# superyuri/FinRL

Hardware: AMD Instinct MI355X
Metric: env-steps/sec at N parallel envs (DOW30, 8 indicators) (higher is better)
Workload: dtype f64

## Files before the change

finrl_amd/csrc/finenv_stocknp.hip:

```cpp

#include <hip/hip_runtime.h>
#include <stdint.h>
#include <stdio.h>
#include <stdlib.h>
#include <string.h>

#include "finenv.h"
#include "finenv_dev.h"
#include "finenv_host.h"

namespace {

constexpr int kWave = 64;
constexpr int kMaxN = FINENV_STOCKNP_MAX_TICKERS;
constexpr int kRowA = kMaxN + 1;
constexpr int kRowH = 2 * kMaxN + 1;
constexpr int kWaves = 4;
constexpr int kLdsPerWave = kWave * kRowH + 2 * kMaxN * kWave + kMaxN;

struct NpParams {
    finenv_stocknp_config cfg;
    finenv_stocknp_panel panel;
    finenv_stocknp_state st;
    const float *actions;
    float *obs;
    float *reward;
    uint8_t *done;
    float *term_obs;
    const uint8_t *mask;
    int32_t auto_reset;
    int32_t D;
    int32_t obs_pitch;
    uint32_t magicN;
    unsigned long long *dbg;
    int32_t diag;
    int32_t *win;
};
struct NpParamsHist : NpParams {
    finenv_stocknp_history hist;
};
template <bool HIST>
using NpArgs = typename std::conditional<HIST, NpParamsHist, NpParams>::type;

#ifdef FINENV_DIAG
#define NDIAG(bit) (p.diag & (bit))
#else
#define NDIAG(bit) 0
#endif

#define NF(fld) (*at(p.st.f64, (unsigned)(fld) * (unsigned)E + (unsigned)e))
#define NI(fld) (*at(p.st.i32, (unsigned)(fld) * (unsigned)E + (unsigned)e))
#define NS(k, i) (*at(p.st.f32, ((unsigned)(k) * (unsigned)N + (unsigned)(i)) * (unsigned)E + (unsigned)e))
#define NWIN(r) (*at(p.win, (unsigned)(r) * (unsigned)E + (unsigned)e))

struct Num { double v; int tag; };
__device__ __forceinline__ Num mk(double v, int tag) { Num r; r.v = v; r.tag = tag; return r; }
__device__ __forceinline__ int promote(int a, int b)
{
    return a == FINENV_NT_PY ? b : (b == FINENV_NT_PY ? a : max(a, b));
}
__device__ __forceinline__ Num n_add(Num a, Num b)
{
    const int t = promote(a.tag, b.tag);
    const double r32 = (double)((float)a.v + (float)b.v), r64 = a.v + b.v;
    return mk(t == FINENV_NT_F32 ? r32 : r64, t);
}
__device__ __forceinline__ Num n_sub(Num a, Num b)
{
    const int t = promote(a.tag, b.tag);
    const double r32 = (double)((float)a.v - (float)b.v), r64 = a.v - b.v;
    return mk(t == FINENV_NT_F32 ? r32 : r64, t);
}
__device__ __forceinline__ Num n_mul(Num a, Num b)
{
    const int t = promote(a.tag, b.tag);
    const double r32 = (double)((float)a.v * (float)b.v), r64 = a.v * b.v;
    return mk(t == FINENV_NT_F32 ? r32 : r64, t);
}
__device__ __forceinline__ Num n_div(Num a, Num b)
{
    const int t = promote(a.tag, b.tag);
    const double r32 = (double)((float)a.v / (float)b.v), r64 = a.v / b.v;
    return mk(t == FINENV_NT_F32 ? r32 : r64, t);
}
__device__ __forceinline__ double floordiv_f32(float a, float b, double q)
{
    const double r = fma(-q, (double)b, (double)a);
    const float mod = (float)((a < 0.0f && r != 0.0) ? r - (double)b : r);
    float div = (a - mod) / b;
    if (mod < 0.0f) div -= 1.0f;
    float fl = floorf(div);
    if (div - fl > 0.5f) fl += 1.0f;
    return (double)fl;
}
__device__ __forceinline__ Num n_floordiv(Num a, Num b)
{
    const int t = promote(a.tag, b.tag);
    const double av = (t == FINENV_NT_F32) ? (double)(float)a.v : a.v;
    const double q = floordiv_true(av, b.v);
    if (t == FINENV_NT_F32 && fabs(q) >= 0x1p22) return mk(floordiv_f32((float)av, (float)b.v, q), t);
    return mk(q, t);
}

__device__ __forceinline__ int scaled_action(float action, float max_stock)
{
    constexpr float kS = 2147483520.0f;
    return (int)__builtin_amdgcn_fmed3f(action * max_stock, -kS, kS);
}

template <bool kCompact = false>
__device__ __forceinline__ void np_write_rows(float *__restrict__ dst, const NpParams &p, int e0,
                                              int nenv_w, int row_day,
                                              unsigned long long lane_mask, const float *heads,
                                              int lane, int k_lo = 0, int k_hi = 1 << 30)
{
    const int N = p.cfg.n_tickers, D = p.D;
    const int pitch = dst == p.obs ? p.obs_pitch : D;
    write_obs_rows_generic<8, 16, kCompact>(
        dst, p.panel.obs_tmpl, D, e0, nenv_w, row_day, lane_mask, heads, kRowH, lane,
        [=](int day, int col) { return day * D + col; },
        [=](int col) {
            const int hidx = col - 3 - N;
            return col == 0 ? 0 : ((hidx >= 0 && hidx < 2 * N) ? 1 + hidx : -1);
        }, k_lo, k_hi, pitch);
}

__device__ __forceinline__ float holdings_value(const float *scol, const float *__restrict__ price,
                                                unsigned pb, int N, const float *prow = nullptr)
{
    if (prow != nullptr) {
        auto prodl = [&](int i) { return scol[i * kWave] * prow[i]; };
        float suml;
        if (N < 8) {
            suml = 0.0f;
            for (int i = 0; i < N; ++i) suml += prodl(i);
        } else {
            float r8[8];
#pragma unroll
            for (int j = 0; j < 8; ++j) r8[j] = prodl(j);
            const int full = N - (N & 7);
            for (int i = 8; i < full; i += 8) {
#pragma unroll
                for (int j = 0; j < 8; ++j) r8[j] += prodl(i + j);
            }
            suml = ((r8[0] + r8[1]) + (r8[2] + r8[3])) + ((r8[4] + r8[5]) + (r8[6] + r8[7]));
            for (int i = full; i < N; ++i) suml += prodl(i);
        }
        return suml;
    }
    auto prod = [&](int i) { return scol[i * kWave] * *at(price, pb + (unsigned)i); };
    float sum;
    if (N < 8) {
        sum = 0.0f;
        for (int i = 0; i < N; ++i) sum += prod(i);
    } else {
        float r8[8];
#pragma unroll
        for (int j = 0; j < 8; ++j) r8[j] = prod(j);
        const int full = N - (N & 7);
        for (int i = 8; i < full; i += 8) {
#pragma unroll
            for (int j = 0; j < 8; ++j) r8[j] += prod(i + j);
        }
        sum = ((r8[0] + r8[1]) + (r8[2] + r8[3])) + ((r8[4] + r8[5]) + (r8[6] + r8[7]));
        for (int i = full; i < N; ++i) sum += prod(i);
    }
    return sum;
}

template <bool RESET_ONLY, bool WIN = false, bool HIST = false>
__global__ void __launch_bounds__(kWave *kWaves *(RESET_ONLY ? 1 : 2)) stocknp_kernel(const NpArgs<HIST> p)
{
    static_assert(!(HIST && RESET_ONLY), "the record is taken by the step");
    __shared__ float lds_all[kWaves * (kLdsPerWave + (HIST ? 2 * kWave : 0))];
    const int lane = threadIdx.x & (kWave - 1);
    const int wib = (threadIdx.x >> 6) % kWaves;
    const int role = (threadIdx.x >> 6) / kWaves;
    float *heads = lds_all + wib * kLdsPerWave;
    float *stk = heads + kWave * kRowH;
    float *cdl = stk + kMaxN * kWave;
    const int E = p.cfg.n_envs, N = p.cfg.n_tickers;
    const int e0 = (blockIdx.x * kWaves + wib) * kWave;
    if (e0 >= E) return;
    const int nenv_w = min(kWave, E - e0);
    const bool valid = lane < nenv_w;
    const int e = valid ? e0 + lane : e0;
    float *scol = stk + lane, *ccol = cdl + lane;
    float *head = heads + lane * kRowH;
    float *prow_lds = cdl + kMaxN * kWave;
    int *hpark = reinterpret_cast<int *>(lds_all + kWaves * kLdsPerWave) + wib * 2 * kWave;

    auto do_reset = [&](Num &amount, Num &ta, Num &gr, Num &ita, int row = 0) {
        for (int i = 0; i < N; ++i) {
            scol[i * kWave] = NS(2, i);
            ccol[i * kWave] = 0.0f;
        }
        amount = mk(NF(FINENV_NF_AMOUNT0), NI(FINENV_NI_AMOUNT0_TAG));
        const unsigned rpb = WIN ? (unsigned)(row * N) : 0u;
        ta = n_add(amount, mk((double)holdings_value(scol, p.panel.price, rpb, N), FINENV_NT_F32));
        ita = ta;
        gr = mk(0.0, FINENV_NT_PY);
    };
    auto fill_head = [&](Num amount) {
        const double fl = p.cfg.obs_amount_floor;
        const Num shown = (fl > 0.0 && fl > amount.v) ? mk(fl, FINENV_NT_PY) : amount;
        head[0] = (float)n_mul(shown, mk(0x1p-12, FINENV_NT_PY)).v;
        for (int i = 0; i < N; ++i) {
            head[1 + i] = scol[i * kWave] * 0x1p-6f;
            head[1 + N + i] = ccol[i * kWave];
        }
    };
    auto store_books = [&](int i_lo, int i_hi) {
        for (int i = i_lo; i < i_hi; ++i) {
            NS(0, i) = scol[i * kWave];
            NS(1, i) = ccol[i * kWave];
        }
    };
    auto store_state = [&](Num amount, Num ta, Num gr, Num ita, int rtag, int day, int i_lo = 0,
                           int i_hi = 1 << 30) {
        NF(FINENV_NF_AMOUNT) = amount.v;
        NF(FINENV_NF_TOTAL_ASSET) = ta.v;
        NF(FINENV_NF_GAMMA_REWARD) = gr.v;
        NF(FINENV_NF_INITIAL_TOTAL_ASSET) = ita.v;
        NI(FINENV_NI_TAGS) = amount.tag | (ta.tag << 2) | (gr.tag << 4) | (ita.tag << 6) | (rtag << 8);
        NI(FINENV_NI_DAY) = day;
        store_books(i_lo, min(i_hi, N));
    };

    if (RESET_ONLY) {
        const bool sel = valid && (p.mask == nullptr || p.mask[e] != 0);
        Num amount, ta, gr, ita;
        int row0 = 0;
        if (WIN) {
            const int ps = NWIN(0), pt = NWIN(1);
            row0 = min(max(ps, 0), p.cfg.n_days - 1);
            if (sel) {
                NWIN(2) = ps;
                NWIN(3) = pt;
            }
        }
        do_reset(amount, ta, gr, ita, row0);
        if (sel) store_state(amount, ta, gr, ita, (NI(FINENV_NI_TAGS) >> 8) & 3, row0);
        if (p.obs == nullptr) return;
        fill_head(amount);
        wave_sync();
        np_write_rows(p.obs, p, e0, nenv_w, row0, __ballot(sel), heads, lane);
        return;
    }

    const int kpatch = (2 + 3 * N) / kWave + 1;
    auto head_widx = [N](int col) {
        const int hidx = col - 3 - N;
        return col == 0 ? 0 : ((hidx >= 0 && hidx < 2 * N) ? 1 + hidx : -1);
    };
    typedef float np_f4 __attribute__((ext_vector_type(4)));
    typedef np_f4 np_f4u __attribute__((aligned(4)));
    const int lpr = 16 * kpatch;
    const bool quad_ok = kpatch <= 2 && p.D >= kWave * kpatch;
    auto head_quads = [&](const np_f4 hq, int el_lo, int el_hi) {
        const int rpi = kWave / lpr, sub = lane / lpr, q = lane & (lpr - 1);
        int w[4];
#pragma unroll
        for (int u = 0; u < 4; ++u) w[u] = head_widx(4 * q + u);
        char *const hb = reinterpret_cast<char *>(p.obs + (size_t)e0 * p.obs_pitch);
        constexpr int kB = 8;
        const int hi = min(nenv_w, el_hi);
        for (int g0 = el_lo / rpi; g0 * rpi < hi; g0 += kB) {
            float pv4[kB][4];
#pragma unroll
            for (int j = 0; j < kB; ++j) {
                const int el = min((g0 + j) * rpi + sub, kWave - 1);
#pragma unroll
                for (int u = 0; u < 4; ++u) pv4[j][u] = heads[el * kRowH + (w[u] >= 0 ? w[u] : 0)];
            }
#pragma unroll
            for (int j = 0; j < kB; ++j) {
                const int el = (g0 + j) * rpi + sub;
                if (el >= hi) continue;
                np_f4 v;
#pragma unroll
                for (int u = 0; u < 4; ++u) v[u] = w[u] >= 0 ? pv4[j][u] : hq[u];
                *reinterpret_cast<np_f4u *>(hb + (size_t)((unsigned)(el * p.obs_pitch + 4 * q) * 4u)) = v;
            }
        }
    };
    auto head_quad_load = [&](int row) -> np_f4 {
        return *reinterpret_cast<const np_f4u *>(reinterpret_cast<const char *>(p.panel.obs_tmpl) +
                                                 (size_t)((unsigned)(row * p.D + 4 * (lane & (lpr - 1))) * 4u));
    };
    if (role == 0) STAMP64(0);
    if (role == 1) {
        int day_s = NI(FINENV_NI_DAY) + 1;
        int last_s = p.cfg.n_days - 1;
        if constexpr (HIST) {
            int hlen_s = *at(p.hist.len, (unsigned)e), hfl_s = *at(p.hist.flags, (unsigned)e);
            if constexpr (WIN) {
                last_s = win_last_day(p.win + 2 * (size_t)E, E, e, p.cfg.n_days);
                asm volatile("s_waitcnt vmcnt(0)"
                             : "+v"(day_s), "+v"(last_s), "+v"(hlen_s), "+v"(hfl_s) : : "memory");
                day_s = min(max(day_s, 0), p.cfg.n_days - 1);
            } else {
                asm volatile("s_waitcnt vmcnt(0)" : "+v"(day_s), "+v"(hlen_s), "+v"(hfl_s) : : "memory");
            }
            hpark[lane] = hlen_s;
            hpark[kWave + lane] = hfl_s;
        } else if constexpr (WIN) {
            last_s = win_last_day(p.win + 2 * (size_t)E, E, e, p.cfg.n_days);
            asm volatile("s_waitcnt vmcnt(0)" : "+v"(day_s), "+v"(last_s) : : "memory");
            day_s = min(max(day_s, 0), p.cfg.n_days - 1);
        } else {
            asm volatile("s_waitcnt vmcnt(0)" : "+v"(day_s) : : "memory");
        }
        lds_barrier();
        const bool done_s = day_s == last_s;
        const unsigned long long vm = __ballot(valid), dm = __ballot(done_s && valid);
        if (dm != 0ull && p.term_obs != nullptr)
            np_write_rows<true>(p.term_obs, p, e0, nenv_w, day_s, dm, heads, lane, kpatch);
        int rd = (done_s && p.auto_reset) ? 0 : day_s;
        if (WIN && p.auto_reset && dm != 0ull) {
            const int ps = win_start(p.win, e, p.cfg.n_days);
            if (done_s) rd = ps;
        }
        const int rd0 = __builtin_amdgcn_readfirstlane(rd);
        const bool same_row = __all(!valid || rd == rd0);
        const bool share = quad_ok && dm == 0ull && same_row;
        np_f4 hq = {0.0f, 0.0f, 0.0f, 0.0f};
        if (share) hq = head_quad_load(rd0);
        STAMP64(9);
        const int c0 = kpatch * kWave, span = p.D - c0;
        if (same_row && span >= 4) {
            const int nq = (span + 3) >> 2;
            char *const ob = reinterpret_cast<char *>(p.obs + (size_t)e0 * p.obs_pitch);
            for (int q0 = 0; q0 < nq; q0 += kWave) {
                const bool qa = q0 + lane < nq;
                const int start = qa ? min(c0 + 4 * (q0 + lane), p.D - 4) : c0;
                const np_f4 t = *reinterpret_cast<const np_f4u *>(
                    reinterpret_cast<const char *>(p.panel.obs_tmpl) + (size_t)((unsigned)(rd0 * p.D + start) * 4u));
#pragma unroll 4
                for (int el = 0; el < nenv_w; ++el)
                    if (qa) *reinterpret_cast<np_f4u *>(ob + (size_t)((unsigned)(el * p.obs_pitch + start) * 4u)) = t;
            }
        } else {
            np_write_rows(p.obs, p, e0, nenv_w, rd, vm, heads, lane, kpatch);
        }
        STAMP64(10);
        lds_barrier();
        if (share && !NDIAG(1)) {
            head_quads(hq, kWave / 2, kWave);
            if (valid) store_books(N / 2, N);
        }
        return;
    }
    int day_ld = NI(FINENV_NI_DAY) + 1;
    int w_last = p.cfg.n_days - 1;
    if (WIN) {
        w_last = win_last_day(p.win + 2 * (size_t)E, E, e, p.cfg.n_days);
        day_ld = min(max(day_ld, 0), p.cfg.n_days - 1);
    }
    const int day = day_ld;
    const int tags = NI(FINENV_NI_TAGS);
    Num amount = mk(NF(FINENV_NF_AMOUNT), tags & 3);
    const Num ta_old = mk(NF(FINENV_NF_TOTAL_ASSET), (tags >> 2) & 3);
    Num gr = mk(NF(FINENV_NF_GAMMA_REWARD), (tags >> 4) & 3);
    Num ita = mk(NF(FINENV_NF_INITIAL_TOTAL_ASSET), (tags >> 6) & 3);
    float sv[kMaxN], cv[kMaxN], av[kMaxN];
#pragma unroll
    for (int i = 0; i < kMaxN; ++i) {
        sv[i] = NS(0, min(i, N - 1));
        cv[i] = NS(1, min(i, N - 1));
    }
    const int a_total = nenv_w * N;
    const float *const a_src = p.actions + (size_t)e0 * N;
#pragma unroll
    for (int j = 0; j < kMaxN; ++j) {
        const int f = j * kWave + lane;
        av[j] = *at(a_src, (unsigned)(f < a_total ? f : a_total - 1));
    }
    const unsigned pb = (unsigned)(day * N);
    const int day0 = __builtin_amdgcn_readfirstlane(day);
    const bool uni = __all(day == day0);
    float prv = 0.0f;
    if (uni && lane < kMaxN) prv = *at(p.panel.price, (unsigned)(day0 * N + min(lane, N - 1)));
    const float *prow = uni ? prow_lds : nullptr;
    np_f4 head_q = {0.0f, 0.0f, 0.0f, 0.0f};
    if (quad_ok) head_q = head_quad_load(day0);
    const bool calm = *at(p.panel.turb_bool, (unsigned)day) == 0.0f;
    lds_barrier();
#pragma unroll
    for (int j = 0; j < kMaxN; ++j) {
        const int f = j * kWave + lane;
        if (f < a_total) {
            const int el = (N == 1) ? f : (int)__umulhi((unsigned)f, p.magicN);
            heads[el * kRowA + (f - el * N)] = av[j];
        }
    }
#pragma unroll
    for (int i = 0; i < kMaxN; ++i) {
        if (i >= N) continue;
        cv[i] += 1.0f;
        scol[i * kWave] = sv[i];
        ccol[i * kWave] = cv[i];
    }
    if (uni && lane < kMaxN) prow_lds[lane] = prv;
    wave_sync();
    STAMP64(1);
    const float *arow = heads + lane * kRowA;
    const float ms = (float)p.cfg.max_stock;
    const Num one_m = mk(1 - p.cfg.sell_cost_pct, FINENV_NT_PY);
    const Num one_p = mk(1 + p.cfg.buy_cost_pct, FINENV_NT_PY);
    const int min_action = p.cfg.min_action;

    constexpr int kPB = 8;
    bool head_filled = false;
    if (__all(amount.tag == FINENV_NT_F64)) {
        double amt = amount.v;
        float (&sr)[kMaxN] = sv, (&cr)[kMaxN] = cv;
        float pr_[kMaxN];
        int ai[kMaxN];
#pragma unroll
        for (int i = 0; i < kMaxN; ++i) {
            const int ic = min(i, N - 1);
            ai[i] = scaled_action(arow[ic], ms);
            pr_[i] = 0.0f;
        }
        if (uni) {
#pragma unroll
            for (int i = 0; i < kMaxN; ++i) pr_[i] = prow_lds[min(i, N - 1)];
        } else {
#pragma unroll
            for (int i = 0; i < kMaxN; ++i) pr_[i] = *at(p.panel.price, pb + (unsigned)min(i, N - 1));
        }
        STAMP64(11);
#pragma unroll
        for (int i = 0; i < kMaxN; ++i) {
            if (i >= N) continue;
            const int a = ai[i];
            const float pr = pr_[i];
            const bool ok = calm && a < -min_action && pr > 0.0f;
            const float s = sr[i];
            const double want = (double)(-a);
            const bool is_int = want < (double)s;
            const double sell = is_int ? want : (double)s;
            const float s_new = (float)((double)s - sell);
            const double t64 = ((double)pr * sell) * one_m.v;
            const double t32 = (double)((pr * (float)sell) * (float)one_m.v);
            const double amt_new = amt + (is_int ? t64 : t32);
            sr[i] = ok ? s_new : s;
            cr[i] = ok ? 0.0f : cr[i];
            amt = ok ? amt_new : amt;
        }
        STAMP64(7);
        double xr[kMaxN];
#pragma unroll
        for (int i = 0; i < kMaxN; ++i) {
            const double d = (double)pr_[i];
            const double x = __builtin_amdgcn_rcp(d);
            xr[i] = fma(fma(-d, x, 1.0), x, x);
        }
        STAMP64(12);
#pragma unroll
        for (int i = 0; i < kMaxN; ++i) {
            if (i >= N) continue;
            const int a = ai[i];
            const double d = (double)pr_[i];
            const bool ok = calm && a > min_action && pr_[i] > 0.0f;
            double q = floor(amt * xr[i]);
            const double r = fma(-q, d, amt);
            q += (r < 0.0) ? -1.0 : ((r >= d) ? 1.0 : 0.0);
            const double buy = ((double)a < q) ? (double)a : q;
            const float s_new = (float)((double)sr[i] + buy);
            const double amt_new = amt - ((d * buy) * one_p.v);
            sr[i] = ok ? s_new : sr[i];
            cr[i] = ok ? 0.0f : cr[i];
            amt = ok ? amt_new : amt;
        }
        amount = mk(amt, FINENV_NT_F64);
        STAMP64(8);
        wave_sync();
        {
            const double fl = p.cfg.obs_amount_floor;
            const Num shown = (fl > 0.0 && fl > amount.v) ? mk(fl, FINENV_NT_PY) : amount;
            head[0] = (float)n_mul(shown, mk(0x1p-12, FINENV_NT_PY)).v;
        }
#pragma unroll
        for (int i = 0; i < kMaxN; ++i) {
            if (i >= N) continue;
            scol[i * kWave] = sr[i];
            ccol[i * kWave] = cr[i];
            head[1 + i] = sr[i] * 0x1p-6f;
            head[1 + N + i] = cr[i];
        }
        head_filled = calm;
    } else {
        for (int i0 = 0; i0 < N; i0 += kPB) {
            float prb[kPB];
    #pragma unroll
            for (int j = 0; j < kPB; ++j) prb[j] = 0.0f;
            if (uni) {
#pragma unroll
                for (int j = 0; j < kPB; ++j) prb[j] = prow_lds[min(i0 + j, N - 1)];
            } else {
#pragma unroll
                for (int j = 0; j < kPB; ++j)
                    prb[j] = *at(p.panel.price, pb + (unsigned)min(i0 + j, N - 1));
            }
    #pragma unroll
            for (int j = 0; j < kPB; ++j) pin(prb[j]);
    #pragma unroll
            for (int j = 0; j < kPB; ++j) {
            const int i = i0 + j;
            if (i >= N) break;
            const int a = scaled_action(arow[i], ms);
            const float pr = prb[j];
            if (calm && a < -min_action && pr > 0.0f) {
                const float s = scol[i * kWave];
                const double want = (double)(-a);
                const bool is_int = want < (double)s;
                const double sell = is_int ? want : (double)s;
                scol[i * kWave] = (float)((double)s - sell);
                const Num t0 = is_int ? mk((double)pr * sell, FINENV_NT_F64)
                                      : mk((double)(pr * (float)sell), FINENV_NT_F32);
                amount = n_add(amount, n_mul(t0, one_m));
                ccol[i * kWave] = 0.0f;
            }
            }
        }
        for (int i0 = 0; i0 < N; i0 += kPB) {
            float prb[kPB];
    #pragma unroll
            for (int j = 0; j < kPB; ++j) prb[j] = 0.0f;
            if (uni) {
#pragma unroll
                for (int j = 0; j < kPB; ++j) prb[j] = prow_lds[min(i0 + j, N - 1)];
            } else {
#pragma unroll
                for (int j = 0; j < kPB; ++j)
                    prb[j] = *at(p.panel.price, pb + (unsigned)min(i0 + j, N - 1));
            }
    #pragma unroll
            for (int j = 0; j < kPB; ++j) pin(prb[j]);
    #pragma unroll
            for (int j = 0; j < kPB; ++j) {
            const int i = i0 + j;
            if (i >= N) break;
            const int a = scaled_action(arow[i], ms);
            const float pr = prb[j];
            if (calm && a > min_action && pr > 0.0f) {
                const Num q = n_floordiv(amount, mk((double)pr, FINENV_NT_F32));
                const bool is_int = (double)a < q.v;
                const double buy = is_int ? (double)a : q.v;
                const Num t0 = is_int ? mk((double)pr * buy, FINENV_NT_F64)
                                      : n_mul(mk((double)pr, FINENV_NT_F32), q);
                const float s = scol[i * kWave];
                scol[i * kWave] = (float)((double)s + buy);
                amount = n_sub(amount, n_mul(t0, one_p));
                ccol[i * kWave] = 0.0f;
            }
            }
        }
    }
    STAMP64(2);
    if (!calm) {
        const Num t0 = mk((double)holdings_value(scol, p.panel.price, pb, N, prow), FINENV_NT_F32);
        amount = n_add(amount, n_mul(t0, one_m));
        for (int i = 0; i < N; ++i) {
            scol[i * kWave] = 0.0f;
            ccol[i * kWave] = 0.0f;
        }
    }
    Num ta = n_add(amount, mk((double)holdings_value(scol, p.panel.price, pb, N, prow), FINENV_NT_F32));
    Num r = n_mul(n_sub(ta, ta_old), mk(p.cfg.reward_scaling, FINENV_NT_PY));
    gr = n_add(n_mul(gr, mk(p.cfg.gamma, FINENV_NT_PY)), r);
    const bool done = day == w_last;
    if (done) {
        r = gr;
        if (valid) NF(FINENV_NF_EPISODE_RETURN) = n_div(ta, ita).v;
    }
    if (valid) {
        *at(p.reward, (unsigned)e) = (float)r.v;
        *at(p.done, (unsigned)e) = done ? 1 : 0;
        NF(FINENV_NF_LAST_REWARD) = r.v;
    }
    if constexpr (HIST) {
        const int hlen = hpark[lane], hfl = hpark[kWave + lane];
        if (valid && hlen >= 1 && !(hfl & FINENV_HIST_COMPLETE)) {
            const bool room = hlen < p.hist.capacity;
            if (room) {
                const size_t o = (size_t)hlen * (size_t)E + (size_t)e;
                p.hist.asset[o] = ta.v;
                if (p.hist.tag != nullptr) p.hist.tag[o] = (uint8_t)ta.tag;
                if (p.hist.stocks != nullptr) {
                    float *const hs = p.hist.stocks + (size_t)hlen * (size_t)N * (size_t)E + (size_t)e;
                    for (int i = 0; i < N; ++i) hs[(size_t)i * (size_t)E] = scol[i * kWave];
                }
                *at(p.hist.len, (unsigned)e) = hlen + 1;
            }
            const int nfl = hfl | (room ? 0 : FINENV_HIST_OVERFLOW) | (done ? FINENV_HIST_COMPLETE : 0);
            if (nfl != hfl) *at(p.hist.flags, (unsigned)e) = nfl;
        }
    }
    STAMP64(3);
    wave_sync();
    if (!head_filled) fill_head(amount);
    wave_sync();
    const unsigned long long valid_mask = __ballot(valid);
    const unsigned long long done_mask = __ballot(done && valid);
    int row_day = day;
    if (done_mask != 0ull) {
        if (p.term_obs != nullptr)
            np_write_rows<true>(p.term_obs, p, e0, nenv_w, day, done_mask, heads, lane, 0, kpatch);
        if (p.auto_reset) {
            wave_sync();
            if (done) {
                if (WIN) {
                    const int ps = NWIN(0), pt = NWIN(1);
                    row_day = min(max(ps, 0), p.cfg.n_days - 1);
                    if (valid) {
                        NWIN(2) = ps;
                        NWIN(3) = pt;
                    }
                } else {
                    row_day = 0;
                }
                do_reset(amount, ta, gr, ita, row_day);
                fill_head(amount);
            }
            wave_sync();
        }
    }
    STAMP64(4);
    const bool share = quad_ok && done_mask == 0ull && __all(!valid || row_day == day0);
    lds_barrier();
    if (!NDIAG(2)) {
        if (share) head_quads(head_q, 0, kWave / 2);
        else np_write_rows(p.obs, p, e0, nenv_w, row_day, valid_mask, heads, lane, 0, kpatch);
    }
    STAMP64(5);
    if (valid) store_state(amount, ta, gr, ita, r.tag, row_day, 0, share ? N / 2 : N);
    STAMP64(6);
}

struct NpHistArgs {
    finenv_stocknp_history h;
    finenv_stocknp_state st;
    const uint8_t *mask;
    int32_t E, N;
};

__global__ __launch_bounds__(256) void stocknp_history_arm_kernel(const NpHistArgs p)
{
    const int E = p.E, N = p.N;
    const int e = blockIdx.x * blockDim.x + threadIdx.x;
    if (e >= E || (p.mask != nullptr && p.mask[e] == 0)) return;
    p.h.asset[e] = NF(FINENV_NF_TOTAL_ASSET);
    if (p.h.tag != nullptr) p.h.tag[e] = (uint8_t)((NI(FINENV_NI_TAGS) >> 2) & 3);
    if (p.h.stocks != nullptr) {
        for (int i = 0; i < N; ++i) p.h.stocks[(size_t)i * (size_t)E + (size_t)e] = NS(0, i);
    }
    p.h.start[e] = NI(FINENV_NI_DAY);
    p.h.len[e] = 1;
    p.h.flags[e] = 0;
}

}

struct finenv_stocknp : finenv_host::Handle {
    finenv_stocknp_config cfg;
    finenv_stocknp_panel panel;
    finenv_stocknp_state st;
    int obs_pitch;
    uint32_t magicN;
    int32_t *win;
    int has_hist;
    finenv_stocknp_history hist;
};

namespace {
NpParams np_params(const finenv_stocknp *h)
{
    NpParams p;
    memset(&p, 0, sizeof(p));
    p.cfg = h->cfg;
    p.panel = h->panel;
    p.st = h->st;
    p.D = h->D;
    p.obs_pitch = h->obs_pitch;
    p.magicN = h->magicN;
    p.win = h->win;
    return p;
}
dim3 np_grid(int E)
{
    const int waves = (E + kWave - 1) / kWave;
    return dim3((unsigned)((waves + kWaves - 1) / kWaves));
}
NpHistArgs np_hist_args(const finenv_stocknp *h)
{
    NpHistArgs a;
    memset(&a, 0, sizeof(a));
    a.h = h->hist;
    a.st = h->st;
    a.E = h->cfg.n_envs;
    a.N = h->cfg.n_tickers;
    return a;
}
void launch_history_arm(const finenv_stocknp *h, const uint8_t *mask, hipStream_t stream)
{
    NpHistArgs a = np_hist_args(h);
    a.mask = mask;
    hipLaunchKernelGGL(stocknp_history_arm_kernel, dim3((a.E + 255) / 256), dim3(256), 0, stream, a);
}
finenv_host::HistorySeries history_series(const finenv_stocknp *h)
{
    return {h->hist.asset, nullptr, nullptr, h->hist.len, h->hist.flags, 0, h->hist.capacity, h->cfg.n_envs};
}
template <bool HIST>
void np_launch_step(const NpArgs<HIST> &p, hipStream_t stream)
{
    const dim3 grid = np_grid(p.cfg.n_envs), block(kWave * kWaves * 2);
    if (p.win != nullptr) hipLaunchKernelGGL((stocknp_kernel<false, true, HIST>), grid, block, 0, stream, p);
    else hipLaunchKernelGGL((stocknp_kernel<false, false, HIST>), grid, block, 0, stream, p);
}
}

extern "C" {

int finenv_stocknp_create(const finenv_stocknp_config *cfg, finenv_stocknp **out)
{
    if (!cfg || !out) return FINENV_ERR_INVALID;
    *out = nullptr;
    if (cfg->n_envs < 1 || cfg->n_tickers < 1 || cfg->n_tickers > FINENV_STOCKNP_MAX_TICKERS ||
        cfg->n_techw < 0 || cfg->n_days < 2 || cfg->min_action < 0 || cfg->max_stock <= 0 ||
        cfg->max_stock > 1e6)
        return FINENV_ERR_INVALID;
    const long long E = cfg->n_envs, N = cfg->n_tickers, T = cfg->n_days;
    const long long D = 3 + 3 * N + cfg->n_techw, lim = (1ll << 32) - 1;
    if (E * 8 * FINENV_STOCKNP_F64_FIELDS > lim || E * N * 12 > lim || T * D * 4 > lim ||
        64 * D * 4 > lim)
        return FINENV_ERR_INVALID;
    finenv_stocknp *h = finenv_host::new_handle<finenv_stocknp>(cfg, D);
    if (!h) return FINENV_ERR_NOMEM;
    h->obs_pitch = (int)D;
    h->magicN = finenv_host::magic_for(N);
    h->win = nullptr;
    *out = h;
    return FINENV_OK;
}

void finenv_stocknp_destroy(finenv_stocknp *h) { delete h; }
const char *finenv_stocknp_last_error(const finenv_stocknp *h) { return finenv_host::last_error(h); }
int finenv_stocknp_obs_dim(const finenv_stocknp *h) { return finenv_host::obs_dim(h); }

int finenv_stocknp_set_obs_pitch(finenv_stocknp *h, int32_t pitch)
{
    if (!h) return FINENV_ERR_INVALID;
    if (pitch == 0) pitch = h->D;
    if (pitch < h->D || (long long)pitch * 64 * 4 > (1ll << 32) - 1)
        return finenv_host::fail(h, FINENV_ERR_INVALID, "set_obs_pitch: pitch must be >= obs_dim");
    h->obs_pitch = pitch;
    return FINENV_OK;
}

int finenv_stocknp_set_windows(finenv_stocknp *h, int32_t *win)
{
    if (!h) return FINENV_ERR_INVALID;
    h->win = win;
    return FINENV_OK;
}

int finenv_stocknp_bind(finenv_stocknp *h, const finenv_stocknp_panel *panel,
                        const finenv_stocknp_state *st)
{
    if (!h || !panel || !st) return FINENV_ERR_INVALID;
    if (!panel->price || !panel->obs_tmpl || !panel->turb_bool || !st->f64 || !st->i32 || !st->f32)
        return finenv_host::fail(h, FINENV_ERR_INVALID, "bind: null pointer");
    return finenv_host::bind(h, panel, st);
}

int finenv_stocknp_reset(finenv_stocknp *h, const uint8_t *mask, float *obs_out, void *stream)
{
    if (const int rc = finenv_host::ready(h, "reset")) return rc;
    const finenv_host::DeviceGuard guard(h->device);
    NpParams p = np_params(h);
    p.mask = mask;
    p.obs = obs_out;
    if (p.win != nullptr)
        hipLaunchKernelGGL((stocknp_kernel<true, true>), np_grid(h->cfg.n_envs), dim3(kWave * kWaves), 0,
                           (hipStream_t)stream, p);
    else
        hipLaunchKernelGGL((stocknp_kernel<true, false>), np_grid(h->cfg.n_envs), dim3(kWave * kWaves), 0,
                           (hipStream_t)stream, p);
    if (h->has_hist) launch_history_arm(h, mask, (hipStream_t)stream);
    return finenv_host::check_launch(h, "stocknp_reset");
}

int finenv_stocknp_step(finenv_stocknp *h, const float *actions, float *obs, float *reward,
                        uint8_t *done, float *term_obs, int32_t auto_reset, void *stream)
{
    if (const int rc = finenv_host::ready(h, "step")) return rc;
    const finenv_host::DeviceGuard guard(h->device);
    if (!actions || !obs || !reward || !done)
        return finenv_host::fail(h, FINENV_ERR_INVALID, "step: null actions/obs/reward/done");
    NpParams p = np_params(h);
    p.actions = actions;
    p.obs = obs;
    p.reward = reward;
    p.done = done;
    p.term_obs = term_obs;
    p.auto_reset = auto_reset;
#ifdef FINENV_DIAG
    p.dbg = g_finenv_dbg;
    {
        const char *d = getenv("FINENV_DIAG");
        p.diag = d ? atoi(d) : 0;
    }
#endif
    if (h->has_hist) {
        NpParamsHist q;
        static_cast<NpParams &>(q) = p;
        q.hist = h->hist;
        np_launch_step<true>(q, (hipStream_t)stream);
    } else {
        np_launch_step<false>(p, (hipStream_t)stream);
    }
    return finenv_host::check_launch(h, "stocknp_step");
}

int finenv_stocknp_set_history(finenv_stocknp *h, const finenv_stocknp_history *hist)
{
    if (!h) return FINENV_ERR_INVALID;
    const bool missing = hist && (!hist->asset || !hist->start || !hist->len || !hist->flags);
    return finenv_host::set_history(h, h->hist, h->has_hist, hist,
                                    missing ? "set_history: null asset/start/len/flags" : nullptr);
}

int finenv_stocknp_history_arm(finenv_stocknp *h, const uint8_t *mask, void *stream)
{
    return finenv_host::history_arm(h, mask, stream, "stocknp_history_arm", launch_history_arm);
}

int finenv_stocknp_history_metrics(finenv_stocknp *h, double annualization, double *out, void *stream)
{
    return finenv_host::history_metrics(h, annualization, out, stream, "stocknp_history_metrics", history_series);
}

}
```

Baseline: 3.561 billion.

## Move template-only head segments into early broadcast store phase

```diff
diff --git a/finrl_amd/csrc/finenv_stocknp.hip b/finrl_amd/csrc/finenv_stocknp.hip
--- a/finrl_amd/csrc/finenv_stocknp.hip
+++ b/finrl_amd/csrc/finenv_stocknp.hip
@@ -125,6 +125,28 @@
         }, k_lo, k_hi, pitch);
 }
 
+__device__ __forceinline__ unsigned clean_head_segments(int N, int D)
+{
+    const int kpatch = (2 + 3 * N) / kWave + 1;
+    unsigned m = 0u;
+    for (int s = 1; s < 4 * kpatch; ++s) {
+        const int lo = 16 * s, hi = lo + 16;
+        if (hi <= D && (hi <= 3 + N || lo >= 3 + 3 * N)) m |= 1u << s;
+    }
+    return m;
+}
+__device__ __forceinline__ int seg_quad_col(unsigned mask, int j)
+{
+    int seg = 0, cnt = 0;
+#pragma unroll
+    for (int b = 0; b < 8; ++b) {
+        const bool set = (mask >> b) & 1u;
+        seg = (set && cnt == (j >> 2)) ? b : seg;
+        cnt += set ? 1 : 0;
+    }
+    return 16 * seg + 4 * (j & 3);
+}
+
 __device__ __forceinline__ float holdings_value(const float *scol, const float *__restrict__ price,
                                                 unsigned pb, int N, const float *prow = nullptr)
 {
@@ -255,38 +277,42 @@
     };
     typedef float np_f4 __attribute__((ext_vector_type(4)));
     typedef np_f4 np_f4u __attribute__((aligned(4)));
-    const int lpr = 16 * kpatch;
-    const bool quad_ok = kpatch <= 2 && p.D >= kWave * kpatch;
+    const int c0 = kpatch * kWave;
+    const bool quad_ok = kpatch <= 2 && p.D >= c0;
+    const unsigned early = (quad_ok && p.D - c0 >= 4) ? clean_head_segments(N, p.D) : 0u;
+    const unsigned late = ((1u << (4 * kpatch)) - 1u) & ~early;
+    const int lpr = 4 * __popc(late);
     auto head_quads = [&](const np_f4 hq, int el_lo, int el_hi) {
-        const int rpi = kWave / lpr, sub = lane / lpr, q = lane & (lpr - 1);
+        const int rpi = kWave / lpr, sub = lane / lpr, col = seg_quad_col(late, lane - sub * lpr);
         int w[4];
 #pragma unroll
-        for (int u = 0; u < 4; ++u) w[u] = head_widx(4 * q + u);
+        for (int u = 0; u < 4; ++u) w[u] = head_widx(col + u);
         char *const hb = reinterpret_cast<char *>(p.obs + (size_t)e0 * p.obs_pitch);
         constexpr int kB = 8;
         const int hi = min(nenv_w, el_hi);
-        for (int g0 = el_lo / rpi; g0 * rpi < hi; g0 += kB) {
+        for (int g0 = el_lo; g0 < hi; g0 += kB * rpi) {
             float pv4[kB][4];
 #pragma unroll
             for (int j = 0; j < kB; ++j) {
-                const int el = min((g0 + j) * rpi + sub, kWave - 1);
+                const int el = min(g0 + j * rpi + sub, kWave - 1);
 #pragma unroll
                 for (int u = 0; u < 4; ++u) pv4[j][u] = heads[el * kRowH + (w[u] >= 0 ? w[u] : 0)];
             }
 #pragma unroll
             for (int j = 0; j < kB; ++j) {
-                const int el = (g0 + j) * rpi + sub;
-                if (el >= hi) continue;
+                const int el = g0 + j * rpi + sub;
+                if (sub >= rpi || el >= hi) continue;
                 np_f4 v;
 #pragma unroll
                 for (int u = 0; u < 4; ++u) v[u] = w[u] >= 0 ? pv4[j][u] : hq[u];
-                *reinterpret_cast<np_f4u *>(hb + (size_t)((unsigned)(el * p.obs_pitch + 4 * q) * 4u)) = v;
+                *reinterpret_cast<np_f4u *>(hb + (size_t)((unsigned)(el * p.obs_pitch + col) * 4u)) = v;
             }
         }
     };
     auto head_quad_load = [&](int row) -> np_f4 {
+        const int col = seg_quad_col(late, lane % lpr);
         return *reinterpret_cast<const np_f4u *>(reinterpret_cast<const char *>(p.panel.obs_tmpl) +
-                                                 (size_t)((unsigned)(row * p.D + 4 * (lane & (lpr - 1))) * 4u));
+                                                 (size_t)((unsigned)(row * p.D + col) * 4u));
     };
     if (role == 0) STAMP64(0);
     if (role == 1) {
@@ -327,13 +353,16 @@
         np_f4 hq = {0.0f, 0.0f, 0.0f, 0.0f};
         if (share) hq = head_quad_load(rd0);
         STAMP64(9);
-        const int c0 = kpatch * kWave, span = p.D - c0;
+        const int span = p.D - c0;
         if (same_row && span >= 4) {
-            const int nq = (span + 3) >> 2;
+            const int nc = share ? 4 * __popc(early) : 0;
+            const int ccol = seg_quad_col(early, lane);
+            const int nq = nc + ((span + 3) >> 2);
             char *const ob = reinterpret_cast<char *>(p.obs + (size_t)e0 * p.obs_pitch);
             for (int q0 = 0; q0 < nq; q0 += kWave) {
-                const bool qa = q0 + lane < nq;
-                const int start = qa ? min(c0 + 4 * (q0 + lane), p.D - 4) : c0;
+                const int q = q0 + lane;
+                const bool qa = q < nq;
+                const int start = !qa ? c0 : (q < nc ? ccol : min(c0 + 4 * (q - nc), p.D - 4));
                 const np_f4 t = *reinterpret_cast<const np_f4u *>(
                     reinterpret_cast<const char *>(p.panel.obs_tmpl) + (size_t)((unsigned)(rd0 * p.D + start) * 4u));
 #pragma unroll 4
```

Measured after the change: 3.526 billion. About the same (-1.0%).
